# monkey0head/RePlay_cql

Measured on NVIDIA B200. Metric: CQL updates/sec (batch 1024), higher is better.
Workload: dtype f32 (f16x3: tensor-core fp16 hi/lo 3-term split with exact power-of-two row scales, fp32 accumulate, 1e-4 parity-gated)

## Files before the change

### replay_cql_b200/csrc/adam_pack.cuh

```cuda
#pragma once
#include "mlp_tc_h2.cuh"

namespace cql {
namespace tc {

struct AdamPackNet {
  float* p;
  float* m;
  float* v;
  const float* g;
  float* targ;
  uint8_t* fwd;
  uint8_t* fwd2;
  uint8_t* bwd;
  uint8_t* bwd2;
  uint8_t* tfwd;
  uint8_t* tfwd2;
  int* w2max;
};
struct AdamPackJobs {
  AdamPackNet n[CQL_MAX_CRITICS];
  int in_dim, out_dim;
  float lr, beta1, beta2, eps, tau;
  long long* step_inc;
  DpPeer dp;
  int dp_group;
  long long dp_off;
};

__device__ __forceinline__ float adam_one(float& p, float& m, float& v, float g, float step_size, float bc2s, float beta1,
                                          float beta2, float eps) {
  const float mi = m + (g - m) * (1.f - beta1);
  const float vi = v * beta2 + (1.f - beta2) * g * g;
  m = mi;
  v = vi;
  p = p - step_size * (mi / (sqrtf(vi) / bc2s + eps));
  return p;
}

__device__ __forceinline__ void store_chunk(const float (&x)[8], float s, uint8_t* one, uint8_t* pair, int n, int kc) {
  uint32_t hi[4], lo[4];
#pragma unroll
  for (int i = 0; i < 4; ++i) split_h2(x[2 * i] * s, x[2 * i + 1] * s, hi[i], lo[i]);
  const uint4 h4 = make_uint4(hi[0], hi[1], hi[2], hi[3]), l4 = make_uint4(lo[0], lo[1], lo[2], lo[3]);
  uint8_t* b = one + (size_t)(n / HCfg::NS) * HCfg::B_BYTES + chunk_off(HCfg::NS, n % HCfg::NS, kc);
  *reinterpret_cast<uint4*>(b) = h4;
  *reinterpret_cast<uint4*>(b + HCfg::B_TERM_BYTES) = l4;
  if (pair != nullptr) {
    *reinterpret_cast<uint4*>(pair + pair_chunk_off(n, kc, 0)) = h4;
    *reinterpret_cast<uint4*>(pair + pair_chunk_off(n, kc, 1)) = l4;
  }
}

constexpr int AP_ROWS = 8;
constexpr int AP_W2_BLOCKS = H / AP_ROWS;

__global__ void __launch_bounds__(1024, 1) k_adam_pack(const AdamPackJobs jobs, const StepInfo* __restrict__ si) {
  grid_dep_wait();
  __shared__ float tile[AP_ROWS][H + 4];
  __shared__ int wm[16];
  const AdamPackNet nt = jobs.n[blockIdx.y];
  const int in_dim = jobs.in_dim, out_dim = jobs.out_dim;
  const float step_size = (float)((double)jobs.lr / si->bc1), bc2s = (float)si->bc2_sqrt;
  const int slot_rd = (int)(si->step % 3), slot_acc = (int)((si->step + 1) % 3), slot_clr = (int)((si->step + 2) % 3);
  const int tid = threadIdx.x, lane = tid & 31;
  const bool dp = jobs.dp.world > 1;
  const long long dpb = jobs.dp_off + (long long)blockIdx.y * NET_STRIDE;
  DpSlices sl{};
  if (dp) {
    sl = dp_slices(jobs.dp, jobs.dp_off, (long long)gridDim.y * NET_STRIDE);
    dp_ll_owner_reduce(jobs.dp, jobs.dp_group, sl, jobs.n[0].g, ((long long)blockIdx.y * gridDim.x + blockIdx.x) * blockDim.x + tid,
                       (long long)gridDim.x * gridDim.y * blockDim.x);
  }
  if (blockIdx.x < AP_W2_BLOCKS) {
    __shared__ float gw2[AP_ROWS][H];
    __shared__ float rmax[AP_ROWS][4], rmaxt[AP_ROWS][4];
    const int r8 = tid >> 7, c2 = tid & 127;
    const int n = blockIdx.x * AP_ROWS + r8;
    const size_t off = (size_t)off_W2(in_dim) + (size_t)n * H + c2 * 2;
    const float w2max_prev = __int_as_float(nt.w2max[slot_rd]);
    float2 g = *reinterpret_cast<const float2*>(nt.g + off);
    float2 m = *reinterpret_cast<const float2*>(nt.m + off), v = *reinterpret_cast<const float2*>(nt.v + off);
    float2 p = *reinterpret_cast<const float2*>(nt.p + off), t = *reinterpret_cast<const float2*>(nt.targ + off);
    if (dp) {
      if ((c2 & 3) == 0) {
        float4 g0 = *reinterpret_cast<const float4*>(nt.g + off), g1 = *reinterpret_cast<const float4*>(nt.g + off + 4);
        dp_ll_mean8(jobs.dp, jobs.dp_group, sl, dpb + (long long)off, g0, g1);
        *reinterpret_cast<float4*>(&gw2[r8][c2 * 2]) = g0;
        *reinterpret_cast<float4*>(&gw2[r8][c2 * 2 + 4]) = g1;
      }
      __syncthreads();
      g = *reinterpret_cast<const float2*>(&gw2[r8][c2 * 2]);
    }
    adam_one(p.x, m.x, v.x, g.x, step_size, bc2s, jobs.beta1, jobs.beta2, jobs.eps);
    adam_one(p.y, m.y, v.y, g.y, step_size, bc2s, jobs.beta1, jobs.beta2, jobs.eps);
    t.x = t.x * (1.f - jobs.tau) + jobs.tau * p.x;
    t.y = t.y * (1.f - jobs.tau) + jobs.tau * p.y;
    *reinterpret_cast<float2*>(nt.m + off) = m;
    *reinterpret_cast<float2*>(nt.v + off) = v;
    *reinterpret_cast<float2*>(nt.p + off) = p;
    *reinterpret_cast<float2*>(nt.targ + off) = t;
    *reinterpret_cast<float2*>(&tile[r8][c2 * 2]) = p;
    float mx = fmaxf(fabsf(p.x), fabsf(p.y)), mt = fmaxf(fabsf(t.x), fabsf(t.y));
#pragma unroll
    for (int o = 16; o > 0; o >>= 1) {
      mx = fmaxf(mx, __shfl_xor_sync(0xffffffffu, mx, o));
      mt = fmaxf(mt, __shfl_xor_sync(0xffffffffu, mt, o));
    }
    if (lane == 0) { rmax[r8][(tid >> 5) & 3] = mx; rmaxt[r8][(tid >> 5) & 3] = mt; }
    __syncthreads();
    mx = fmaxf(fmaxf(rmax[r8][0], rmax[r8][1]), fmaxf(rmax[r8][2], rmax[r8][3]));
    mt = fmaxf(fmaxf(rmaxt[r8][0], rmaxt[r8][1]), fmaxf(rmaxt[r8][2], rmaxt[r8][3]));
    float s, inv_s, st, inv_st;
    pow2_scale(mx, s, inv_s);
    pow2_scale(mt, st, inv_st);
    {
// ... 9 lines not shown
      if (nt.fwd2 != nullptr) {
        *reinterpret_cast<uint32_t*>(nt.fwd2 + pair_chunk_off(n, kc, 0) + piece) = hi;
        *reinterpret_cast<uint32_t*>(nt.fwd2 + pair_chunk_off(n, kc, 1) + piece) = lo;
      }
      if (nt.tfwd2 != nullptr) {
        *reinterpret_cast<uint32_t*>(nt.tfwd2 + pair_chunk_off(n, kc, 0) + piece) = thi;
        *reinterpret_cast<uint32_t*>(nt.tfwd2 + pair_chunk_off(n, kc, 1) + piece) = tlo;
      }
    }
    if (c2 == 0) {
      reinterpret_cast<HMeta*>(nt.fwd + HCfg::META_OFF)->inv_s[n] = inv_s;
      reinterpret_cast<HMeta*>(nt.tfwd + HCfg::META_OFF)->inv_s[n] = inv_st;
      if (nt.fwd2) reinterpret_cast<HMeta*>(nt.fwd2 + H2Cfg::META_OFF)->inv_s[n] = inv_s;
      if (nt.tfwd2) reinterpret_cast<HMeta*>(nt.tfwd2 + H2Cfg::META_OFF)->inv_s[n] = inv_st;
      atomicMax(&nt.w2max[slot_acc], __float_as_int(mx));
    }
    if (tid < H) {
      const float bound = 2.f * (w2max_prev + 4.f * jobs.lr);
      float sT, inv_sT;
      pow2_scale(bound, sT, inv_sT);
      const int np = tid;
      float x[8];
#pragma unroll
      for (int i = 0; i < 8; ++i) x[i] = tile[i][np];
      store_chunk(x, sT, nt.bwd, nt.bwd2, np, (int)blockIdx.x);
      if (blockIdx.x == 0) {
        reinterpret_cast<HMeta*>(nt.bwd + HCfg::META_OFF)->inv_s[np] = inv_sT;
        if (nt.bwd2) reinterpret_cast<HMeta*>(nt.bwd2 + H2Cfg::META_OFF)->inv_s[np] = inv_sT;
      }
    }
    if (dp) dp_consume_done(jobs.dp, jobs.dp_group, gridDim.x * gridDim.y);
    return;
  }
  if (tid >= 256) return;
  if (tid < 16) wm[tid] = 0;
  if (tid == 0) nt.w2max[slot_clr] = 0;
  __syncthreads();
  __shared__ float gsm[2048];
  const int w2_lo = off_W2(in_dim), w2_hi = w2_lo + H * H;
  if (dp) {
    {
      const int c = tid * 8;
      const int idx = c < w2_lo ? c : c + H * H;
      if (idx + 7 < NET_STRIDE) {
        float4 a = *reinterpret_cast<const float4*>(nt.g + idx), b = *reinterpret_cast<const float4*>(nt.g + idx + 4);
        dp_ll_mean8(jobs.dp, jobs.dp_group, sl, dpb + idx, a, b);
        *reinterpret_cast<float4*>(gsm + c) = a;
        *reinterpret_cast<float4*>(gsm + c + 4) = b;
      }
    }
    __syncthreads();
  }
  auto grad_of = [&](int idx) { return dp ? gsm[idx < w2_lo ? idx : idx - H * H] : nt.g[idx]; };
  const int k = tid;
  int idxs[8];
  int n_idx = 0;
  for (int c = 0; c < in_dim; ++c) idxs[n_idx++] = off_W1(in_dim) + k * in_dim + c;
  idxs[n_idx++] = off_b1(in_dim) + k;
  idxs[n_idx++] = off_b2(in_dim) + k;
  for (int o = 0; o < out_dim; ++o) idxs[n_idx++] = off_W3(in_dim) + o * H + k;
  const bool has_b3 = tid < out_dim;
  const int ib3 = off_b3(in_dim, out_dim) + tid;
  float gv[9], pv[9], mv[9], vv[9], tv[9];
#pragma unroll
  for (int i = 0; i < 8; ++i)
    if (i < n_idx) { gv[i] = grad_of(idxs[i]); pv[i] = nt.p[idxs[i]]; mv[i] = nt.m[idxs[i]]; vv[i] = nt.v[idxs[i]]; tv[i] = nt.targ[idxs[i]]; }
  if (has_b3) { gv[8] = grad_of(ib3); pv[8] = nt.p[ib3]; mv[8] = nt.m[ib3]; vv[8] = nt.v[ib3]; tv[8] = nt.targ[ib3]; }
#pragma unroll
  for (int i = 0; i < 9; ++i)
    if (i < n_idx || (i == 8 && has_b3)) {
      adam_one(pv[i], mv[i], vv[i], gv[i], step_size, bc2s, jobs.beta1, jobs.beta2, jobs.eps);
// ... 52 lines not shown
```

### replay_cql_b200/csrc/capi.cu

```cuda
#include <cstring>
#include <cstdio>
#include <algorithm>
#include "engine.cuh"
#include "update.cuh"
#include "score.cuh"
#include "tc_selftest.cuh"
#include "score_tc.cuh"
#include "score_tc_h.cuh"
#include "topk_staged.cuh"
#include "metrics.cuh"
#include "dp_peer.cuh"
#include "mma_bench.cuh"

using namespace cql;

struct cql_handle {
  Handle h;
  cudaGraphExec_t graph_exec = nullptr;
  cudaStream_t graph_stream = nullptr;
  int64_t graph_launches = 0;
  cudaGraphExec_t batch_graph[2] = {nullptr, nullptr};
  cudaStream_t batch_graph_stream[2] = {nullptr, nullptr};
  int64_t batch_graph_launches[2] = {0, 0};
  void* sbuf[8] = {nullptr, nullptr, nullptr, nullptr, nullptr, nullptr, nullptr, nullptr};
// ... 155 lines not shown
  h.XT = h.dalloc<float4>(B);
  h.QT = h.dalloc<float>((size_t)C * B);
  h.XP = h.dalloc<float4>(B);
  h.QP = h.dalloc<float>((size_t)C * B);
  h.h2P = h.dalloc<float>((size_t)C * tB * H * BM);
  h.dQP = h.dalloc<float>((size_t)C * B);
  h.dXP = h.dalloc<float4>((size_t)C * B);
  h.dOutA = h.dalloc<float>(2 * (size_t)B);
  h.perb = h.dalloc<float>(4 * (size_t)B);
  h.pairv = h.dalloc<float>(4 * (size_t)C * B);
  h.loss_sums = h.dalloc<float>(16);
  h.actor_part = h.dalloc<float>((size_t)((B + 127) / 128) * 4 + 4);
  h.splitsC = std::max(1, std::min(tC, (2 * h.num_sms) / (4 * C)));
  h.splitsA = std::max(1, std::min(tB, (2 * h.num_sms) / 4));
  h.smallC = h.dalloc<float>((size_t)C * tC * SMALL_STRIDE);
  h.smallA = h.dalloc<float>((size_t)tB * SMALL_STRIDE);
  h.pw2C = h.dalloc<float>((size_t)C * h.splitsC * H * H);
  h.pw2A = h.dalloc<float>((size_t)h.splitsA * H * H);
  if (cfg->precision != CQL_PREC_FP32) {
    const bool bf = cfg->precision == CQL_PREC_BF16, f16 = cfg->precision == CQL_PREC_F16X3;
    h.packed_net_bytes = f16 ? tc::HCfg::PACKED_NET_BYTES : (bf ? tc::Cfg<false>::PACKED_NET_BYTES : tc::Cfg<true>::PACKED_NET_BYTES);
    h.packed_net_bytes_bwd = f16 ? tc::HCfg::PACKED_NET_BYTES : (bf ? tc::Cfg<false>::PACKED_NET_BYTES : tc::Cfg<true>::PACKED_NET_BYTES);
    h.packed_fwd = h.dalloc<uint8_t>((size_t)(2 + 2 * C) * h.packed_net_bytes);
    const int slices = f16 ? tc::HCfg::SLICES : (bf ? tc::Cfg<false>::SLICES : tc::Cfg<true>::SLICES);
    h.part_floats = (size_t)C * std::max(slices, (int)tc::H2Cfg::PARTS) * ((size_t)B * (2 * n3 + 2)) * 2 + 4096;
    h.part = h.dalloc<float>(h.part_floats);
    h.tc_slices = slices;
    h.packed_bwd = h.dalloc<uint8_t>((size_t)(1 + C) * h.packed_net_bytes_bwd);
    if (f16) {
      h.packed_net_bytes2 = tc::H2Cfg::PACKED_NET_BYTES;
      h.packed_fwd2 = h.dalloc<uint8_t>((size_t)(2 + 2 * C) * h.packed_net_bytes2);
      h.packed_bwd2 = h.dalloc<uint8_t>((size_t)(1 + C) * h.packed_net_bytes2);
      h.w2max = h.dalloc<int>((size_t)(2 + 2 * C) * 4);
      if (const char* sw = std::getenv("CQL_PAIR_SWAP")) h.pair_swap_b = std::atoi(sw);
    }
    h.slots1 = (f16 ? tc::HCfg::NEW : 4) * h.num_sms;
    h.splits_tc = h.num_sms;
    h.small1 = h.dalloc<float>((size_t)C * h.slots1 * SMALL_STRIDE);
    h.small2 = h.dalloc<float>((size_t)C * h.splits_tc * SMALL_STRIDE);
    h.pw2_tc = h.dalloc<float>((size_t)(h.num_sms + C) * H * H);
    h.dX_part = h.dalloc<float4>((size_t)C * std::max(slices, 8) * B);
    h.b2_tickets = h.dalloc<unsigned int>((size_t)CQL_MAX_CRITICS * 64 + 64);
  }
  float sc[SCALAR_SLOT] = {0};
  sc[0] = logf(cfg->initial_temperature);
  sc[1] = logf(cfg->initial_alpha);
  CQL_CUDA(cudaMemcpy(h.scalars(), sc, sizeof(sc), cudaMemcpyHostToDevice));
}

void destroy_graph(cql_handle* ch) {
  if (ch->graph_exec) { cudaGraphExecDestroy(ch->graph_exec); ch->graph_exec = nullptr; }
  for (auto& g : ch->batch_graph) if (g) { cudaGraphExecDestroy(g); g = nullptr; }
  if (ch->step_graph) { cudaGraphExecDestroy(ch->step_graph); ch->step_graph = nullptr; }
}

template <typename F>
int guarded(cql_handle* ch, F&& f) {
  if (!ch) { g_create_error = "NULL handle"; return 1; }
  struct DeviceScope {
    int prev = -1;
    ~DeviceScope() { if (prev >= 0) cudaSetDevice(prev); }
  } scope;
  try {
    int cur = -1;
    if (cudaGetDevice(&cur) == cudaSuccess && cur != ch->h.cfg.device) scope.prev = cur;
    CQL_CUDA(cudaSetDevice(ch->h.cfg.device));
// ... 856 lines not shown
```

### replay_cql_b200/csrc/engine.cuh

```cuda
#pragma once
#include <vector>
#include <string>
#include "common.cuh"
#include "mlp_simt.cuh"
#include "dp_peer.cuh"
#include <nvtx3/nvToolsExt.h>

namespace cql {

constexpr int N_NOISE_PARTS = 8;

struct StepInfo {
  double bc1, bc2_sqrt;
  long long step;
};

struct NvtxRange {
  explicit NvtxRange(const char* name) { nvtxRangePushA(name); }
  ~NvtxRange() { nvtxRangePop(); }
  NvtxRange(const NvtxRange&) = delete;
  NvtxRange& operator=(const NvtxRange&) = delete;
};

struct MdpSession;
// ... 45 lines not shown
  float* h2C = nullptr;
  float* dQ = nullptr;
  float4* XT = nullptr;
  float* QT = nullptr;
  float4* XP = nullptr;
  float* QP = nullptr;
  float* h2P = nullptr;
  float* dQP = nullptr;
  float4* dXP = nullptr;
  float* dOutA = nullptr;
  float* perb = nullptr;
  float* pairv = nullptr;
  float* loss_sums = nullptr;
  float* actor_part = nullptr;
  float* smallC = nullptr;
  float* smallA = nullptr;
  float* pw2C = nullptr;
  float* pw2A = nullptr;
  int splitsC = 1, splitsA = 1;

  uint8_t* packed_fwd = nullptr;
  size_t packed_net_bytes = 0;
  size_t packed_net_bytes_bwd = 0;
  float* part = nullptr;
  size_t part_floats = 0;
  uint8_t* packed_bwd = nullptr;
  float* small1 = nullptr;
  float* small2 = nullptr;
  float* pw2_tc = nullptr;
  float4* dX_part = nullptr;
  unsigned int* b2_tickets = nullptr;
  int slots1 = 0, splits_tc = 0, tc_slices = 1;
  int last_dx_parts = 0;
  uint8_t* packed_fwd2 = nullptr;
  uint8_t* packed_bwd2 = nullptr;
  size_t packed_net_bytes2 = 0;
  DpPeer dp;
  bool dp_fused = false;
  int* w2max = nullptr;
  int pair_swap_b = 0;

  bool timing = false;
  cudaEvent_t ev[16] = {};

  MdpSession* mdp = nullptr;
  uint8_t* mdp_ring = nullptr;
  std::vector<void*> allocs;

  template <typename T>
  T* dalloc(size_t count) {
    void* p = nullptr;
    CQL_CUDA(cudaMalloc(&p, count * sizeof(T)));
    CQL_CUDA(cudaMemset(p, 0, count * sizeof(T)));
    allocs.push_back(p);
    return reinterpret_cast<T*>(p);
  }
  void free_all() {
    for (void* p : allocs) cudaFree(p);
    allocs.clear();
    if (mdp) { mdp_session_free(mdp); mdp = nullptr; }
    if (mdp_ring) { cudaFreeHost(mdp_ring); mdp_ring = nullptr; }
    if (table) { cudaFree(table); table = nullptr; table_cap = 0; }
    if (metrics_host) { cudaFreeHost(metrics_host); metrics_host = nullptr; }
    if (batch_host) { cudaFreeHost(batch_host); batch_host = nullptr; }
    if (noise_host) { cudaFreeHost(noise_host); noise_host = nullptr; }
    if (own_stream) { cudaStreamDestroy(own_stream); own_stream = nullptr; }
    if (side_stream) { cudaStreamDestroy(side_stream); side_stream = nullptr; }
    if (ev_fork) { cudaEventDestroy(ev_fork); ev_fork = nullptr; }
    if (ev_join) { cudaEventDestroy(ev_join); ev_join = nullptr; }
    for (auto& e : ev) if (e) { cudaEventDestroy(e); e = nullptr; }
  }

// ... 36 lines not shown
```

### replay_cql_b200/csrc/mlp_tc_bwd1.cuh

```cuda
#pragma once
#include "mlp_tc.cuh"
#include "mlp_tc_ts.cuh"

namespace cql {
namespace tc {

struct Bwd1Job {
  const float4* X;
  const float* dOut;
  const float* h2;
  const float* params;
  const uint8_t* packedT;
  float* small1;
  float4* dX_part;
  int rows, n_nets, slots;
  const float* q_part = nullptr;
  int q_parts = 0;
  float dq_scale = 0.f;
};
template <int IN, int OUT>
__device__ __forceinline__ float actor_dq_of(const Bwd1Job& jb, int net_i, int r) {
  constexpr int MAXP = 8;
  int arg = 0;
  float qm = 0.f;
  for (int c = 0; c < jb.n_nets; ++c) {
    float part[MAXP];
#pragma unroll
    for (int p = 0; p < MAXP; ++p)
      if (p < jb.q_parts) part[p] = __ldg(jb.q_part + ((size_t)c * jb.q_parts + p) * jb.rows + r);
    const float bias = __ldg(jb.params + (size_t)c * NET_STRIDE + off_b3(IN, OUT));
    float v = 0.f;
#pragma unroll
    for (int p = 0; p < MAXP; ++p)
      if (p < jb.q_parts) v += part[p];
    const float q = v + bias;
    if (c == 0 || q < qm) { qm = q; arg = c; }
  }
  return net_i == arg ? jb.dq_scale : 0.f;
}

__device__ __forceinline__ float warp_reduce_scatter32(float (&v)[32]) {
  const int lane = threadIdx.x & 31;
#pragma unroll
  for (int off = 16; off >= 1; off >>= 1) {
    const bool upper = (lane & off) != 0;
#pragma unroll
    for (int i = 0; i < off; ++i) {
      const float send = upper ? v[i] : v[i + off];
      const float keep = upper ? v[i + off] : v[i];
      v[i] = keep + __shfl_xor_sync(0xffffffffu, send, off);
    }
  }
// ... 465 lines not shown
      tc_fence_before();
      __syncwarp();
      if (lane == 0) mbar_arrive(&tempty[acc]);
      if (DX && row < jb.rows)
        jb.dX_part[((size_t)net_i * C::SLICES + slice) * jb.rows + row] = make_float4(dx0, dx1, dx2, 0.f);
      ++tcount;
    }
    flush(cur_pair);
  }
  tc_fence_before();
  __syncthreads();
  if (warp == C::MMA_WARP) tmem_dealloc(tmem, C::TMEM_ALLOC);
}

__device__ __forceinline__ float4 sum_strided4(const float* __restrict__ p, int n, size_t stride) {
  float4 s0 = make_float4(0.f, 0.f, 0.f, 0.f), s1 = s0, s2 = s0, s3 = s0;
  int i = 0;
  for (; i + 4 <= n; i += 4) {
    const float4 a = __ldg(reinterpret_cast<const float4*>(p + (size_t)i * stride));
    const float4 b = __ldg(reinterpret_cast<const float4*>(p + (size_t)(i + 1) * stride));
    const float4 c = __ldg(reinterpret_cast<const float4*>(p + (size_t)(i + 2) * stride));
    const float4 d = __ldg(reinterpret_cast<const float4*>(p + (size_t)(i + 3) * stride));
    s0.x += a.x; s0.y += a.y; s0.z += a.z; s0.w += a.w;
    s1.x += b.x; s1.y += b.y; s1.z += b.z; s1.w += b.w;
    s2.x += c.x; s2.y += c.y; s2.z += c.z; s2.w += c.w;
    s3.x += d.x; s3.y += d.y; s3.z += d.z; s3.w += d.w;
  }
  for (; i < n; ++i) {
    const float4 a = __ldg(reinterpret_cast<const float4*>(p + (size_t)i * stride));
    s0.x += a.x; s0.y += a.y; s0.z += a.z; s0.w += a.w;
  }
  return make_float4((s0.x + s1.x) + (s2.x + s3.x), (s0.y + s1.y) + (s2.y + s3.y), (s0.z + s1.z) + (s2.z + s3.z),
                     (s0.w + s1.w) + (s2.w + s3.w));
}

__global__ void __launch_bounds__(256) k_reduce_grads_tc(const float* __restrict__ small1, int slots1,
                                                         const float* __restrict__ small2, const float* __restrict__ pw2,
                                                         int splits, int in_dim, int out_dim, float* __restrict__ grads,
                                                         int w2_group = 1, const DpPeer dp = DpPeer{}, int dp_group = 0,
                                                         long long dp_off = 0) {
  tc::grid_dep_wait();
 
  __shared__ float4 part[8][32];
  const int net = blockIdx.y;
  const int g = threadIdx.x & 31, chunk = threadIdx.x >> 5;
  const int idx = (blockIdx.x * 32 + g) * 4;
  const int w2_lo = off_W2(in_dim), w2_hi = w2_lo + H * H, total = net_floats(in_dim, out_dim);
  float4 s = make_float4(0.f, 0.f, 0.f, 0.f);
  if (idx < NET_STRIDE) {
    const float* base = nullptr;
    int n = 0;
    size_t stride = 0;
    if (idx >= w2_lo && idx < w2_hi) {
      base = pw2 + (size_t)net * splits * H * H + (idx - w2_lo); n = (splits + w2_group - 1) / w2_group; stride = (size_t)w2_group * H * H;
    } else if (idx < w2_lo) {
      base = small1 + (size_t)net * slots1 * SMALL_STRIDE + idx; n = slots1; stride = SMALL_STRIDE;
    } else if (idx < total) {
      base = small2 + (size_t)net * splits * SMALL_STRIDE + (idx - H * H); n = splits; stride = SMALL_STRIDE;
    }
    const int per = (n + 7) / 8, lo = chunk * per, hi = min(n, lo + per);
    if (base != nullptr && hi > lo) s = sum_strided4(base + (size_t)lo * stride, hi - lo, stride);
  }
  part[chunk][g] = s;
  __syncthreads();
  if (chunk == 0 && idx < NET_STRIDE) {
    float4 t = part[0][g];
// ... 11 lines not shown
```

### replay_cql_b200/csrc/mlp_tc_h.cuh

```cuda
#pragma once
#include <cuda_fp16.h>
#include "mlp_tc.cuh"
#include "mlp_tc_bwd1.cuh"
#include "mlp_tc_bwd2.cuh"

namespace cql {
namespace tc {

template <int NEW_, int NS_ = 128>
struct HCfgT {
  static constexpr int ES = 2, EPC = 8, UK = 16;
  static constexpr int NS = NS_;
  static constexpr int SLICES = H / NS;
  static constexpr int NPW = 16;
  static constexpr int KC = 64;
  static constexpr int STAGES = 4;
  static constexpr int NCHUNK = H / KC;
  static constexpr int KPW = KC / (NPW / 4);
  static constexpr int NEW = NEW_;
  static constexpr int MMA_WARP = NEW + NPW;
  static constexpr int THREADS = (NEW + 1 + NPW) * 32;
  static constexpr int PROD_THREADS = NPW * 32;
  static constexpr uint32_t B_TERM_BYTES = NS * H * ES;
  static constexpr uint32_t B_BYTES = 2 * B_TERM_BYTES;
// ... 401 lines not shown
  float4* ebs = reinterpret_cast<float4*>(sm + C::OFF_EB);
  float* invs = reinterpret_cast<float*>(sm + C::OFF_W1 + H * 8);
  uint64_t* bars = reinterpret_cast<uint64_t*>(sm + C::OFF_BAR);
  uint64_t* full = bars;
  uint64_t* empty = bars + C::STAGES;
  uint64_t* tfull = bars + 2 * C::STAGES;
  uint64_t* tempty = tfull + 2;
  uint64_t* bload = tempty + 2;
  uint64_t* drain = bload + 1;
  uint32_t* slot = reinterpret_cast<uint32_t*>(sm + C::OFF_SLOT);

  const int tid = threadIdx.x, warp = tid >> 5, lane = tid & 31;
  const int tiles = (jb.rows + TM - 1) / TM;
  const int tiles64 = (jb.rows + 63) / 64;
  const int total = jb.n_nets * C::SLICES * tiles;
  const int item_lo = (int)((long long)total * blockIdx.x / gridDim.x);
  const int item_hi = (int)((long long)total * (blockIdx.x + 1) / gridDim.x);

  if (warp == C::MMA_WARP) {
    tmem_alloc(slot, C::TMEM_ALLOC);
    if (lane == 0) {
      for (int s = 0; s < C::STAGES; ++s) { mbar_init(&full[s], C::NPW); mbar_init(&empty[s], 1); }
      for (int q = 0; q < 2; ++q) { mbar_init(&tfull[q], 1); mbar_init(&tempty[q], 4); }
      mbar_init(bload, 1);
      mbar_init(drain, 1);
      fence_mbar_init();
    }
  }
  tc_fence_before();
  __syncthreads();
  tc_fence_after();
  const uint32_t tmem = *slot;
  grid_dep_wait();

  if (warp == C::MMA_WARP) {
    const uint32_t idesc = instr_desc(FMT_F16, TM, C::NS);
    const uint32_t b_lbo = C::NS * 16;
    const uint32_t b_base = smem_u32(Bs);
    int cur_pair = -1;
    uint32_t it = 0, nb = 0, nd = 0, tcount = 0;
    for (int item = item_lo; item < item_hi; ++item) {
      const int pair = item / tiles;
      if (pair != cur_pair) {
        if (cur_pair >= 0) { if (elect_one()) umma_commit(drain); __syncwarp(); mbar_wait(drain, nd & 1); ++nd; }
        if (elect_one()) load_operand_slice<C>(Bs, jb.packedT + (size_t)(pair / C::SLICES) * HCfg::PACKED_NET_BYTES, pair % C::SLICES, bload);
        __syncwarp();
        mbar_wait(bload, nb & 1);
        ++nb;
        cur_pair = pair;
      }
      const uint32_t acc = tcount & 1;
      mbar_wait(&tempty[acc], ((tcount >> 1) & 1) ^ 1);
      tc_fence_after();
      const uint32_t d_tmem = tmem + acc * C::NS;
      for (int c = 0; c < C::NCHUNK; ++c, ++it) {
        const uint32_t s = it % C::STAGES;
        mbar_wait(&full[s], (it / C::STAGES) & 1);
        tc_fence_after();
        if (elect_one()) {
          const uint32_t a_stage = tmem + C::A_COL0 + s * C::A_STAGE_COLS;
#pragma unroll
          for (int j = 0; j < C::KC / C::UK; ++j) {
            const uint32_t g = c * (C::KC / C::UK) + j;
            const uint64_t b_hi = smem_desc(b_base + 2 * g * b_lbo, b_lbo, 128);
            const uint64_t b_lo = smem_desc(b_base + C::B_TERM_BYTES + 2 * g * b_lbo, b_lbo, 128);
            const uint32_t a_hi = a_stage + j * 8, a_lo = a_hi + C::A_LO_COLS;
// ... 494 lines not shown
```

### replay_cql_b200/csrc/mlp_tc_h2.cuh

```cuda
#pragma once
#include "mlp_tc_h.cuh"

namespace cql {
namespace tc {

__device__ __forceinline__ uint32_t cluster_ctarank() {
  uint32_t r;
  asm volatile("mov.u32 %0, %%cluster_ctarank;" : "=r"(r));
  return r;
}
__device__ __forceinline__ void cluster_sync_all() {
  asm volatile("barrier.cluster.arrive.release.aligned;" ::: "memory");
  asm volatile("barrier.cluster.wait.acquire.aligned;" ::: "memory");
}
__device__ __forceinline__ void mbar_arrive_cluster(uint64_t* bar, uint32_t cta) {
  asm volatile(
      "{\n\t.reg .b32 ra;\n\tmapa.shared::cluster.u32 ra, %0, %1;\n\t"
      "mbarrier.arrive.shared::cluster.b64 _, [ra];\n\t}" ::"r"(smem_u32(bar)),
      "r"(cta)
      : "memory");
}
__device__ __forceinline__ void mbar_wait_cluster(uint64_t* bar, uint32_t parity) { mbar_wait(bar, parity); }
__device__ __forceinline__ void tmem_alloc2(uint32_t* smem_slot, uint32_t ncols) {
  asm volatile("tcgen05.alloc.cta_group::2.sync.aligned.shared::cta.b32 [%0], %1;" ::"r"(smem_u32(smem_slot)), "r"(ncols)
// ... 443 lines not shown
  uint64_t* tempty = tfull + 2;
  uint64_t* bload = tempty + 2;
  uint64_t* bready = bload + 1;
  uint64_t* drain = bready + 1;
  uint32_t* slot = reinterpret_cast<uint32_t*>(sm + C::OFF_SLOT);

  const int tid = threadIdx.x, warp = tid >> 5, lane = tid & 31;
  const uint32_t rank = cluster_ctarank();
  const bool leader = rank == 0;
  const int cluster_id = blockIdx.x >> 1, n_clusters = gridDim.x >> 1;
  const int tiles = pair_tiles(jb.rows);
  const int tiles64 = (jb.rows + 63) / 64;
  const int total = jb.n_nets * tiles;
  const int item_lo = (int)((long long)total * cluster_id / n_clusters);
  const int item_hi = (int)((long long)total * (cluster_id + 1) / n_clusters);

  if (warp == C::MMA_WARP) {
    tmem_alloc2(slot, 512);
    if (lane == 0) {
      for (int s = 0; s < C::STAGES; ++s) { mbar_init(&full[s], 2 * C::NPW); mbar_init(&empty[s], 1); }
      for (int a = 0; a < 2; ++a) { mbar_init(&tfull[a], 1); mbar_init(&tempty[a], 2 * C::NEW); }
      mbar_init(bload, 1);
      mbar_init(bready, 2);
      mbar_init(drain, 1);
      fence_mbar_init();
    }
  }
  tc_fence_before();
  __syncthreads();
  cluster_sync_all();
  tc_fence_after();
  const uint32_t tmem = *slot;
  grid_dep_wait();

  if (warp == C::MMA_WARP) {
    const uint32_t idesc = instr_desc(FMT_F16, C::TMP, C::NP);
    const uint32_t b_lbo = C::NLOC * 16;
    const uint32_t b_base = smem_u32(Bs);
    int cur_net = -1;
    uint32_t nb = 0, nd = 0, tcount = 0;
    for (int item = item_lo; item < item_hi; ++item) {
      const int net_i = item / tiles;
      if (net_i != cur_net) {
        if (cur_net >= 0) {
          if (leader && elect_one()) umma_commit2(drain, 3);
          __syncwarp();
          mbar_wait_cluster(drain, nd & 1);
          ++nd;
        }
        const uint8_t* src = jb.packedT + (size_t)net_i * C::PACKED_NET_BYTES + (size_t)(rank ^ (uint32_t)swap_b) * C::B_BYTES;
        if (elect_one()) {
          mbar_arrive_expect_tx(bload, C::B_BYTES);
          for (uint32_t o = 0; o < C::B_BYTES; o += 32768) bulk_g2s(Bs + o, src + o, 32768, bload);
        }
        __syncwarp();
        mbar_wait(bload, nb & 1);
        if (elect_one()) mbar_arrive_cluster(bready, 0);
        __syncwarp();
        if (leader) mbar_wait_cluster(bready, nb & 1);
        ++nb;
        cur_net = net_i;
      }
      if (!leader) continue;
      for (int p = 0; p < C::PASSES; ++p) {
        mbar_wait_cluster(&tempty[p], (tcount & 1) ^ 1);
        tc_fence_after();
// ... 545 lines not shown
```

### replay_cql_b200/csrc/update.cuh

```cuda
#pragma once
#include <algorithm>
#include <utility>
#include <cstdlib>
#include "engine.cuh"
#include "mlp_tc.cuh"
#include "mlp_tc_ts.cuh"
#include <type_traits>
#include "mlp_tc_bwd1.cuh"
#include "mlp_tc_bwd2.cuh"
#include "mlp_tc_h.cuh"
#include "mlp_tc_h2.cuh"
#include "adam_pack.cuh"

namespace cql {

__host__ __device__ inline uint32_t mix32(uint32_t x) {
  x ^= x >> 16; x *= 0x7feb352du; x ^= x >> 15; x *= 0x846ca68bu; x ^= x >> 16;
  return x;
}
__host__ __device__ inline uint64_t feistel_perm(uint64_t x, uint64_t n, uint64_t key) {
  int bits = 2;
  while (bits < 62 && (1ull << bits) < n) bits += 2;
  const int hb = bits / 2;
  const uint64_t mask = (1ull << hb) - 1;
// ... 703 lines not shown
  }
  if (jobs_h.n) {
    launch_pdl(tc::k_pack_multi_h, dim3(dim3(H * 32 / 256, jobs_h.n)), dim3(256), 0, st, jobs_h, 2);
    CQL_LAUNCH_CHECK(h);
    tc::PackJobs jp{};
    for (int i = 0; i < n_slots; ++i) {
      const int slot = slots[i];
      const bool is_actor = slot == slot_actor() || slot == slot_targ_actor(h->C);
      if (is_actor) continue;
      jp.j[jp.n++] = {h->net_params(slot), h->packed_fwd2 + (size_t)slot * h->packed_net_bytes2, 3, 0};
      if (slot <= h->C) jp.j[jp.n++] = {h->net_params(slot), h->packed_bwd2 + (size_t)slot * h->packed_net_bytes2, 3, 1};
    }
    if (jp.n) {
      launch_pdl(tc::k_pack_pair_h, dim3(dim3(H * 32 / 256, jp.n)), dim3(256), 0, st, jp, 2);
      CQL_LAUNCH_CHECK(h);
    }
  }
  if (jobs.n == 0) return;
  if (h->cfg.precision != CQL_PREC_BF16) {
    const int chunks = H * (H / tc::Cfg<true>::EPC);
    tc::k_pack_multi<true><<<dim3((chunks + 255) / 256, jobs.n), 256, 0, st>>>(jobs);
  } else {
    const int chunks = H * (H / tc::Cfg<false>::EPC);
    tc::k_pack_multi<false><<<dim3((chunks + 255) / 256, jobs.n), 256, 0, st>>>(jobs);
  }
  CQL_LAUNCH_CHECK(h);
}
inline void pack_weights(Handle* h, int slot, int n_slots, int , cudaStream_t st) {
  int slots[8];
  for (int i = 0; i < n_slots; ++i) slots[i] = slot + i;
  pack_slots(h, slots, n_slots, st);
}

template <bool TF32, int IN, int OUT, bool WGRADS, bool DX, bool F16X3 = false>
inline void launch_bwd_tc(Handle* h, const BwdJob& jb, float* grads_out, cudaStream_t st, int mark_mid = -1, int mark_end = -1) {
  using C = std::conditional_t<F16X3, tc::HCfg, tc::Cfg<TF32>>;
  const int slot = (int)((jb.params - h->params) / NET_STRIDE);
  const int tiles = (jb.rows + tc::TM - 1) / tc::TM;
  const int items = jb.n_nets * C::SLICES * tiles;
  bool pair = false;
  if constexpr (F16X3) {
    static const bool no_pair = std::getenv("CQL_NO_PAIR") != nullptr || std::getenv("CQL_NO_PAIR_BWD1") != nullptr;
    pair = !no_pair && IN == 3 && jb.n_nets * ((jb.rows + 2 * tc::TM - 1) / (2 * tc::TM)) >= h->num_sms / 2;
  }
  bool small = false;
  if constexpr (F16X3) {
    static const bool no_small = std::getenv("CQL_NO_SMALL") != nullptr;
    small = !pair && !no_small && items * 2 <= h->num_sms;
  }
  const int n_slices = small ? tc::HCfgS::SLICES : C::SLICES;
  const int items_s = jb.n_nets * n_slices * tiles;
  static const bool no_fork = std::getenv("CQL_NO_FORK") != nullptr;
  static const int big_fork = std::getenv("CQL_BIG_FORK") ? std::atoi(std::getenv("CQL_BIG_FORK")) : -1;
  const int fork_pairs = big_fork >= 0 ? big_fork : (h->num_sms / 2) * 30 / 74;
  const int clusters1 = (pair && WGRADS && fork_pairs > 0 && fork_pairs < h->num_sms / 2 && !no_fork && !h->timing && h->side_stream != nullptr)
                            ? fork_pairs : h->num_sms / 2;
  const int grid1 = pair ? 2 * clusters1 : (items_s < h->num_sms ? items_s : h->num_sms);
  h->last_dx_parts = jb.n_nets * (pair ? (int)tc::H2Cfg::PARTS : n_slices);
  const int slots1 = (F16X3 ? 2 : 4) * grid1;
  if (WGRADS) CQL_CUDA(cudaMemsetAsync(h->small1, 0, (size_t)jb.n_nets * slots1 * SMALL_STRIDE * sizeof(float), st));
  tc::Bwd1Job j1{jb.X, jb.dOut, jb.h2, jb.params,
                 pair ? h->packed_bwd2 + (size_t)slot * h->packed_net_bytes2 : h->packed_bwd + (size_t)slot * h->packed_net_bytes_bwd,
                 h->small1, DX ? h->dX_part : nullptr, jb.rows, jb.n_nets, slots1};
  j1.q_part = jb.q_part; j1.q_parts = jb.q_parts; j1.dq_scale = jb.dq_scale;
  constexpr int RS2 = F16X3 ? tc::B2HCfg::RS : tc::B2Cfg<TF32>::RS;
  const int n_stage = (jb.rows + RS2 - 1) / RS2;
  int splits = h->num_sms / jb.n_nets;
  if (splits > n_stage) splits = n_stage;
  if (splits > h->splits_tc) splits = h->splits_tc;
  if (splits < 1) splits = 1;
  bool pair2 = false;
  if constexpr (F16X3) {
    static const bool no_pair2 = std::getenv("CQL_NO_PAIR") != nullptr || std::getenv("CQL_NO_PAIR_BWD2") != nullptr;
    static const bool no_pair2_small = std::getenv("CQL_NO_PAIR_BWD2_SMALL") != nullptr;
    pair2 = !no_pair2 && (pair || !no_pair2_small);
    if (pair2) splits = std::max(1, std::min(n_stage, (h->num_sms / 2) / jb.n_nets));
    if (pair2 && pair && clusters1 < h->num_sms / 2) splits = std::max(1, (h->num_sms / 2 - clusters1) / jb.n_nets);
  }
  const bool fork = WGRADS && !no_fork && !h->timing && h->side_stream != nullptr &&
                    grid1 + (pair2 ? 2 : 1) * splits * jb.n_nets <= h->num_sms;
  cudaStream_t st2 = st;
  if (fork) {
    CQL_CUDA(cudaEventRecord(h->ev_fork, st));
    CQL_CUDA(cudaStreamWaitEvent(h->side_stream, h->ev_fork, 0));
    st2 = h->side_stream;
  }
  if constexpr (F16X3) {
    if (pair) launch_pdl_pair(tc::tc_bwd1_h2_kernel<IN, OUT, WGRADS, DX>, clusters1, dim3(tc::H2Cfg::THREADS), tc::H2B1Cfg::SMEM_BYTES, st, j1, h->pair_swap_b);
    else if (small) launch_pdl(tc::tc_bwd1_h_kernel<IN, OUT, WGRADS, DX, tc::HCfgS>, dim3(grid1), dim3(tc::HCfgS::THREADS), tc::HCfgS::SMEM_BYTES, st, j1);
    else launch_pdl(tc::tc_bwd1_h_kernel<IN, OUT, WGRADS, DX>, dim3(grid1), dim3(tc::HCfg::THREADS), tc::HCfg::SMEM_BYTES, st, j1);
  } else if constexpr (TF32)
    tc::tc_bwd1_ts_kernel<IN, OUT, WGRADS, DX><<<grid1, tc::TsCfg::THREADS, tc::TsCfg::SMEM_BYTES, st>>>(j1);
  else
    tc::tc_bwd1_kernel<TF32, IN, OUT, WGRADS, DX><<<grid1, tc::Pipe<TF32, tc::BWD1_NPW>::THREADS, tc::FwdSmem<TF32, tc::BWD1_NPW>::BYTES, st>>>(j1);
  CQL_LAUNCH_CHECK(h);
  if (mark_mid >= 0) mark(h, st, mark_mid);
  if (!WGRADS) return;
  tc::Bwd2Job j2{jb.X, jb.dOut, jb.h2, jb.params, h->pw2_tc, h->small2, jb.rows, jb.n_nets, splits};
  constexpr bool GROUP_SUM = false;
  if (F16X3 && GROUP_SUM) j2.tickets = h->b2_tickets;
  if constexpr (F16X3) {
    if (pair2) {
      static const bool no_pdl_env = std::getenv("CQL_NO_PDL") != nullptr;
      cudaLaunchConfig_t cfg{};
      cfg.gridDim = dim3(2 * splits, jb.n_nets); cfg.blockDim = dim3(tc::B2PCfg::THREADS); cfg.dynamicSmemBytes = tc::B2PCfg::BYTES; cfg.stream = st2;
      cudaLaunchAttribute attr[1];
      attr[0].id = cudaLaunchAttributeProgrammaticStreamSerialization;
      attr[0].val.programmaticStreamSerializationAllowed = 1;
      cfg.attrs = attr;
      cfg.numAttrs = (no_pdl_env || g_timing_no_pdl) ? 0 : 1;
      CQL_CUDA(cudaLaunchKernelEx(&cfg, tc::tc_bwd2_h2_kernel<IN, OUT>, j2));
    } else {
      launch_pdl(tc::tc_bwd2_h_kernel<IN, OUT>, dim3(splits, jb.n_nets), dim3(tc::B2HCfg::THREADS), tc::B2HCfg::BYTES, st2, j2);
    }
  } else
    tc::tc_bwd2_kernel<TF32, IN, OUT><<<dim3(splits, jb.n_nets), tc::B2_THREADS, tc::B2Cfg<TF32>::BYTES, st2>>>(j2);
  CQL_LAUNCH_CHECK(h);
  if (fork) {
    CQL_CUDA(cudaEventRecord(h->ev_join, st2));
    CQL_CUDA(cudaStreamWaitEvent(st, h->ev_join, 0));
  }
  if (mark_end >= 0) mark(h, st, mark_end);
  if (!skip_launch(64))
    launch_pdl(tc::k_reduce_grads_tc, dim3(dim3((NET_STRIDE / 4 + 31) / 32, jb.n_nets)), dim3(256), 0, st, h->small1, slots1, h->small2, h->pw2_tc,
                                                                                  splits, IN, OUT, grads_out,
                                                                                  (F16X3 && GROUP_SUM) ? tc::B2H_GROUP : 1,
                                                                                  h->dp_fused ? h->dp : DpPeer{}, IN == 3 ? 1 : 2,
                                                                                  (long long)(IN == 3 ? NET_STRIDE : 0));
  CQL_LAUNCH_CHECK(h);
}

inline void adam_pack(Handle* h, int first_slot, int n_nets, int in_dim, int out_dim, float lr, cudaStream_t st, bool last = false) {
  const cql_config& c = h->cfg;
  tc::AdamPackJobs j{};
  j.in_dim = in_dim; j.out_dim = out_dim;
  j.lr = lr; j.beta1 = c.beta1; j.beta2 = c.beta2; j.eps = c.adam_eps; j.tau = c.tau;
  j.step_inc = last ? h->step_dev : nullptr;
  j.dp = h->dp_fused ? h->dp : DpPeer{};
  j.dp_group = in_dim == 3 ? 1 : 2;
  j.dp_off = (long long)first_slot * NET_STRIDE;
  for (int i = 0; i < n_nets; ++i) {
    const int slot = first_slot + i, tslot = slot + 1 + h->C;
    const bool critic = in_dim == 3;
    tc::AdamPackNet& n = j.n[i];
    n.p = h->net_params(slot);
    n.m = h->adam_m + (size_t)slot * NET_STRIDE;
    n.v = h->adam_v + (size_t)slot * NET_STRIDE;
    n.g = h->grads + (size_t)slot * NET_STRIDE;
    n.targ = h->net_params(tslot);
    n.fwd = h->packed_fwd + (size_t)slot * h->packed_net_bytes;
    n.bwd = h->packed_bwd + (size_t)slot * h->packed_net_bytes_bwd;
    n.tfwd = h->packed_fwd + (size_t)tslot * h->packed_net_bytes;
    n.fwd2 = critic ? h->packed_fwd2 + (size_t)slot * h->packed_net_bytes2 : nullptr;
    n.bwd2 = critic ? h->packed_bwd2 + (size_t)slot * h->packed_net_bytes2 : nullptr;
    n.tfwd2 = critic ? h->packed_fwd2 + (size_t)tslot * h->packed_net_bytes2 : nullptr;
    n.w2max = h->w2max + slot * 4;
  }
  if (!skip_launch(128))
    launch_pdl(tc::k_adam_pack, dim3(tc::AP_W2_BLOCKS + 1, n_nets), dim3(1024), 0, st, j, h->stepinfo);
  CQL_LAUNCH_CHECK(h);
}

inline void pack_all_weights(Handle* h, cudaStream_t st) {
  if (h->cfg.precision == CQL_PREC_F16X3) {
    tc::k_w2max_init<<<2 + 2 * h->C, 256, 0, st>>>(h->params, 2 + 2 * h->C, h->w2max);
    CQL_LAUNCH_CHECK(h);
  }
  pack_weights(h, slot_actor(), 1, 2, st);
  pack_weights(h, slot_critic(0), h->C, 3, st);
  pack_weights(h, slot_targ_actor(h->C), 1, 2, st);
  pack_weights(h, slot_targ_critic(h->C, 0), h->C, 3, st);
}

template <int IN, int OUT, bool WGRADS, bool DX>
inline void launch_bwd1(Handle* h, const BwdJob& jb, cudaStream_t st) {
  mlp_bwd1_kernel<IN, OUT, WGRADS, DX><<<tiles_of(jb.rows) * jb.n_nets, NT, BWD1_SMEM, st>>>(jb);
  CQL_LAUNCH_CHECK(h);
}

template <int IN, int OUT>
inline void launch_bwd2(Handle* h, const BwdJob& jb, cudaStream_t st) {
  mlp_bwd2_kernel<IN, OUT><<<dim3(4, jb.splits, jb.n_nets), NT, BWD2_SMEM, st>>>(jb);
  CQL_LAUNCH_CHECK(h);
}

inline LossConsts loss_consts(const Handle* h) {
  const cql_config& c = h->cfg;
  return LossConsts{h->B, h->n, h->C, c.gamma, c.conservative_weight, c.alpha_threshold,
                    c.temp_lr, c.alpha_lr, c.beta1, c.beta2, c.adam_eps};
}

constexpr int TIMED_FWD_REPS = 4;
// ... 195 lines not shown
```

Baseline: 4600.

## Fold gradient partial reduction into Adam-pack kernel and zero slots in bwd1

The separate k_reduce_grads_tc launch is dropped in the f16x3 single-device path. The Adam-pack kernel now sums the per-split W2 partials and the small-parameter slot partials itself, writes the gradient, and applies Adam. Small parameters are spread over many blocks, with a ticket-based last-block reduction for the weight maxima that go into the packed metadata. The cudaMemset of the small1 slots is replaced by zeroing inside the bwd1 kernel. This saves a kernel launch, a memset and a round trip of the gradients through global memory, at the cost of extra cross-block atomics and more work inside the Adam kernel.

```diff
diff --git a/replay_cql_b200/csrc/adam_pack.cuh b/replay_cql_b200/csrc/adam_pack.cuh
--- a/replay_cql_b200/csrc/adam_pack.cuh
+++ b/replay_cql_b200/csrc/adam_pack.cuh
@@ -8,7 +8,7 @@
   float* p;
   float* m;
   float* v;
-  const float* g;
+  float* g;
   float* targ;
   uint8_t* fwd;
   uint8_t* fwd2;
@@ -26,6 +26,11 @@
   DpPeer dp;
   int dp_group;
   long long dp_off;
+  const float* small1;
+  const float* small2;
+  const float* pw2;
+  int slots1, splits;
+  int* wmax_acc;
 };
 
 __device__ __forceinline__ float adam_one(float& p, float& m, float& v, float g, float step_size, float bc2s, float beta1,
@@ -54,10 +59,81 @@
 
 constexpr int AP_ROWS = 8;
 constexpr int AP_W2_BLOCKS = H / AP_ROWS;
+constexpr int AP_SMALL_E = 128;
+constexpr int ap_small_blocks(int in_dim, int out_dim) { return (net_floats(in_dim, out_dim) - H * H + AP_SMALL_E - 1) / AP_SMALL_E; }
+
+__device__ __forceinline__ void adam_small_fold(const AdamPackJobs& jobs, const AdamPackNet& nt, float step_size, float bc2s,
+                                             int slot_clr, int* wm) {
+  __shared__ float part[8][AP_SMALL_E];
+  __shared__ int last;
+  const int tid = threadIdx.x, in_dim = jobs.in_dim, out_dim = jobs.out_dim;
+  const int w2_lo = off_W2(in_dim), n_e = net_floats(in_dim, out_dim) - H * H;
+  const int s_blk = blockIdx.x - AP_W2_BLOCKS, n_blk = gridDim.x - AP_W2_BLOCKS;
+  const int el = tid % AP_SMALL_E, chunk = tid / AP_SMALL_E;
+  const int e = s_blk * AP_SMALL_E + el;
+  const int idx = e < w2_lo ? e : e + H * H;
+  const bool own = tid < AP_SMALL_E && e < n_e;
+  float p = 0.f, m = 0.f, v = 0.f, t = 0.f;
+  if (own) { p = nt.p[idx]; m = nt.m[idx]; v = nt.v[idx]; t = nt.targ[idx]; }
+  float s = 0.f;
+  if (e < n_e) {
+    if (e < w2_lo) s = chunk_sum8<float, 16>(jobs.small1 + (size_t)blockIdx.y * jobs.slots1 * SMALL_STRIDE + e, jobs.slots1, SMALL_STRIDE, chunk);
+    else s = chunk_sum8<float, 16>(jobs.small2 + (size_t)blockIdx.y * jobs.splits * SMALL_STRIDE + e, jobs.splits, SMALL_STRIDE, chunk);
+  }
+  part[chunk][el] = s;
+  if (tid < 16) wm[tid] = 0;
+  if (s_blk == 0 && tid == 0) {
+    nt.w2max[slot_clr] = 0;
+    if (jobs.step_inc != nullptr && blockIdx.y == 0) *jobs.step_inc += 1;
+  }
+  __syncthreads();
+  if (own) {
+    float g = part[0][el];
+#pragma unroll
+    for (int c = 1; c < 8; ++c) g += part[c][el];
+    nt.g[idx] = g;
+    m = __fmaf_rn(__fsub_rn(g, m), __fsub_rn(1.f, jobs.beta1), m);
+    v = __fmaf_rn(g, __fmul_rn(g, __fsub_rn(1.f, jobs.beta2)), __fmul_rn(jobs.beta2, v));
+    p = __fmaf_rn(-__fdiv_rn(m, __fadd_rn(__fdiv_rn(__fsqrt_rn(v), bc2s), jobs.eps)), step_size, p);
+    t = __fmaf_rn(t, __fsub_rn(1.f, jobs.tau), __fmul_rn(jobs.tau, p));
+    nt.p[idx] = p; nt.m[idx] = m; nt.v[idx] = v; nt.targ[idx] = t;
+    int slot = -1;
+    if (idx < off_b1(in_dim)) slot = idx % in_dim;
+    else if (idx < w2_lo) slot = 3;
+    else if (idx >= off_W3(in_dim) && idx < off_b3(in_dim, out_dim)) slot = 4 + (idx - off_W3(in_dim)) / H;
+    if (slot >= 0) {
+      atomicMax(&wm[slot], __float_as_int(fabsf(p)));
+      atomicMax(&wm[8 + slot], __float_as_int(fabsf(t)));
+    }
+  }
+  __syncthreads();
+  int* acc = jobs.wmax_acc + blockIdx.y * 16;
+  unsigned int* ticket = reinterpret_cast<unsigned int*>(jobs.wmax_acc + CQL_MAX_CRITICS * 16) + blockIdx.y;
+  if (tid < 16 && wm[tid] != 0) atomicMax(&acc[tid], wm[tid]);
+  __threadfence();
+  __syncthreads();
+  if (tid == 0) {
+    const unsigned int k = atomicAdd(ticket, 1u);
+    last = k == (unsigned int)n_blk - 1;
+    if (last) *ticket = 0;
+  }
+  __syncthreads();
+  if (!last) return;
+  __threadfence();
+  if (tid < 8) {
+    const float w = __int_as_float(atomicExch(&acc[tid], 0)), wt = __int_as_float(atomicExch(&acc[8 + tid], 0));
+    reinterpret_cast<HMeta*>(nt.fwd + HCfg::META_OFF)->wmax[tid] = w;
+    reinterpret_cast<HMeta*>(nt.bwd + HCfg::META_OFF)->wmax[tid] = w;
+    reinterpret_cast<HMeta*>(nt.tfwd + HCfg::META_OFF)->wmax[tid] = wt;
+    if (nt.fwd2) reinterpret_cast<HMeta*>(nt.fwd2 + H2Cfg::META_OFF)->wmax[tid] = w;
+    if (nt.bwd2) reinterpret_cast<HMeta*>(nt.bwd2 + H2Cfg::META_OFF)->wmax[tid] = w;
+    if (nt.tfwd2) reinterpret_cast<HMeta*>(nt.tfwd2 + H2Cfg::META_OFF)->wmax[tid] = wt;
+  }
+}
 
 __global__ void __launch_bounds__(1024, 1) k_adam_pack(const AdamPackJobs jobs, const StepInfo* __restrict__ si) {
   grid_dep_wait();
-  __shared__ float tile[AP_ROWS][H + 4];
+  __shared__ __align__(16) float tile[AP_ROWS][H + 4];
   __shared__ int wm[16];
   const AdamPackNet nt = jobs.n[blockIdx.y];
   const int in_dim = jobs.in_dim, out_dim = jobs.out_dim;
@@ -73,15 +149,21 @@
                        (long long)gridDim.x * gridDim.y * blockDim.x);
   }
   if (blockIdx.x < AP_W2_BLOCKS) {
-    __shared__ float gw2[AP_ROWS][H];
+    __shared__ __align__(16) float gw2[AP_ROWS][H];
     __shared__ float rmax[AP_ROWS][4], rmaxt[AP_ROWS][4];
     const int r8 = tid >> 7, c2 = tid & 127;
     const int n = blockIdx.x * AP_ROWS + r8;
     const size_t off = (size_t)off_W2(in_dim) + (size_t)n * H + c2 * 2;
     const float w2max_prev = __int_as_float(nt.w2max[slot_rd]);
-    float2 g = *reinterpret_cast<const float2*>(nt.g + off);
+    float2 g;
+    if (jobs.small1 == nullptr) g = *reinterpret_cast<const float2*>(nt.g + off);
     float2 m = *reinterpret_cast<const float2*>(nt.m + off), v = *reinterpret_cast<const float2*>(nt.v + off);
     float2 p = *reinterpret_cast<const float2*>(nt.p + off), t = *reinterpret_cast<const float2*>(nt.targ + off);
+    if (jobs.small1 != nullptr) {
+      g = reduce8<float2, 4>(jobs.pw2 + (size_t)blockIdx.y * jobs.splits * H * H + (off - off_W2(in_dim)), jobs.splits,
+                             (size_t)H * H);
+      *reinterpret_cast<float2*>(nt.g + off) = g;
+    }
     if (dp) {
       if ((c2 & 3) == 0) {
         float4 g0 = *reinterpret_cast<const float4*>(nt.g + off), g1 = *reinterpret_cast<const float4*>(nt.g + off + 4);
@@ -157,11 +239,15 @@
     if (dp) dp_consume_done(jobs.dp, jobs.dp_group, gridDim.x * gridDim.y);
     return;
   }
+  if (jobs.small1 != nullptr) {
+    adam_small_fold(jobs, nt, step_size, bc2s, slot_clr, wm);
+    return;
+  }
   if (tid >= 256) return;
   if (tid < 16) wm[tid] = 0;
   if (tid == 0) nt.w2max[slot_clr] = 0;
   __syncthreads();
-  __shared__ float gsm[2048];
+  __shared__ __align__(16) float gsm[2048];
   const int w2_lo = off_W2(in_dim), w2_hi = w2_lo + H * H;
   if (dp) {
     {
diff --git a/replay_cql_b200/csrc/capi.cu b/replay_cql_b200/csrc/capi.cu
--- a/replay_cql_b200/csrc/capi.cu
+++ b/replay_cql_b200/csrc/capi.cu
@@ -211,6 +211,7 @@
       h.packed_fwd2 = h.dalloc<uint8_t>((size_t)(2 + 2 * C) * h.packed_net_bytes2);
       h.packed_bwd2 = h.dalloc<uint8_t>((size_t)(1 + C) * h.packed_net_bytes2);
       h.w2max = h.dalloc<int>((size_t)(2 + 2 * C) * 4);
+      h.ap_wmax = h.dalloc<int>((size_t)CQL_MAX_CRITICS * 17);
       if (const char* sw = std::getenv("CQL_PAIR_SWAP")) h.pair_swap_b = std::atoi(sw);
     }
     h.slots1 = (f16 ? tc::HCfg::NEW : 4) * h.num_sms;
diff --git a/replay_cql_b200/csrc/engine.cuh b/replay_cql_b200/csrc/engine.cuh
--- a/replay_cql_b200/csrc/engine.cuh
+++ b/replay_cql_b200/csrc/engine.cuh
@@ -101,12 +101,14 @@
   unsigned int* b2_tickets = nullptr;
   int slots1 = 0, splits_tc = 0, tc_slices = 1;
   int last_dx_parts = 0;
+  int last_slots1 = 0, last_splits = 0;
   uint8_t* packed_fwd2 = nullptr;
   uint8_t* packed_bwd2 = nullptr;
   size_t packed_net_bytes2 = 0;
   DpPeer dp;
   bool dp_fused = false;
   int* w2max = nullptr;
+  int* ap_wmax = nullptr;
   int pair_swap_b = 0;
 
   bool timing = false;
diff --git a/replay_cql_b200/csrc/mlp_tc_bwd1.cuh b/replay_cql_b200/csrc/mlp_tc_bwd1.cuh
--- a/replay_cql_b200/csrc/mlp_tc_bwd1.cuh
+++ b/replay_cql_b200/csrc/mlp_tc_bwd1.cuh
@@ -17,7 +17,19 @@
   const float* q_part = nullptr;
   int q_parts = 0;
   float dq_scale = 0.f;
+  int zero_small1 = 0;
 };
+template <int IN>
+__device__ __forceinline__ void zero_small1_slots(const Bwd1Job& jb, int per_cta) {
+  if (!jb.zero_small1) return;
+  constexpr int NF4 = off_W2(IN) / 4;
+  for (int net = 0; net < jb.n_nets; ++net)
+    for (int s = 0; s < per_cta; ++s) {
+      float4* o = reinterpret_cast<float4*>(jb.small1 + ((size_t)net * jb.slots + (size_t)blockIdx.x * per_cta + s) * SMALL_STRIDE);
+      for (int f = threadIdx.x; f < NF4; f += blockDim.x) o[f] = make_float4(0.f, 0.f, 0.f, 0.f);
+    }
+  __syncthreads();
+}
 template <int IN, int OUT>
 __device__ __forceinline__ float actor_dq_of(const Bwd1Job& jb, int net_i, int r) {
   constexpr int MAXP = 8;
@@ -549,6 +561,54 @@
   }
   return make_float4((s0.x + s1.x) + (s2.x + s3.x), (s0.y + s1.y) + (s2.y + s3.y), (s0.z + s1.z) + (s2.z + s3.z),
                      (s0.w + s1.w) + (s2.w + s3.w));
+}
+
+__device__ __forceinline__ void vacc(float& s, float a) { s += a; }
+__device__ __forceinline__ void vacc(float2& s, float2 a) { s.x += a.x; s.y += a.y; }
+__device__ __forceinline__ float vfold(float a, float b, float c, float d) { return (a + b) + (c + d); }
+__device__ __forceinline__ float2 vfold(float2 a, float2 b, float2 c, float2 d) {
+  return make_float2((a.x + b.x) + (c.x + d.x), (a.y + b.y) + (c.y + d.y));
+}
+template <typename V> __device__ __forceinline__ V vld(const float* p);
+template <> __device__ __forceinline__ float vld<float>(const float* p) { return __ldg(p); }
+template <> __device__ __forceinline__ float2 vld<float2>(const float* p) { return __ldg(reinterpret_cast<const float2*>(p)); }
+template <typename V, int NPRE>
+__device__ __forceinline__ V sum_strided_pre(const float* __restrict__ p, int n, size_t stride) {
+  static_assert(NPRE % 4 == 0, "groups of four");
+  V s0{}, s1{}, s2{}, s3{};
+  if (n <= NPRE) {
+    V a[NPRE];
+#pragma unroll
+    for (int i = 0; i < NPRE; ++i)
+      if (i < n) a[i] = vld<V>(p + (size_t)i * stride);
+#pragma unroll
+    for (int i = 0; i < NPRE; i += 4)
+      if (i + 4 <= n) { vacc(s0, a[i]); vacc(s1, a[i + 1]); vacc(s2, a[i + 2]); vacc(s3, a[i + 3]); }
+#pragma unroll
+    for (int i = 0; i < NPRE; ++i)
+      if (i >= (n & ~3) && i < n) vacc(s0, a[i]);
+  } else {
+    int i = 0;
+    for (; i + 4 <= n; i += 4) {
+      const V a = vld<V>(p + (size_t)i * stride), b = vld<V>(p + (size_t)(i + 1) * stride);
+      const V c = vld<V>(p + (size_t)(i + 2) * stride), d = vld<V>(p + (size_t)(i + 3) * stride);
+      vacc(s0, a); vacc(s1, b); vacc(s2, c); vacc(s3, d);
+    }
+    for (; i < n; ++i) vacc(s0, vld<V>(p + (size_t)i * stride));
+  }
+  return vfold(s0, s1, s2, s3);
+}
+template <typename V, int NPRE>
+__device__ __forceinline__ V chunk_sum8(const float* __restrict__ p, int n, size_t stride, int chunk) {
+  const int per = (n + 7) / 8, lo = chunk * per, hi = min(n, lo + per);
+  return hi > lo ? sum_strided_pre<V, NPRE>(p + (size_t)lo * stride, hi - lo, stride) : V{};
+}
+template <typename V, int NPRE>
+__device__ __forceinline__ V reduce8(const float* __restrict__ p, int n, size_t stride) {
+  V t = chunk_sum8<V, NPRE>(p, n, stride, 0);
+#pragma unroll
+  for (int c = 1; c < 8; ++c) vacc(t, chunk_sum8<V, NPRE>(p, n, stride, c));
+  return t;
 }
 
 __global__ void __launch_bounds__(256) k_reduce_grads_tc(const float* __restrict__ small1, int slots1,
diff --git a/replay_cql_b200/csrc/mlp_tc_h.cuh b/replay_cql_b200/csrc/mlp_tc_h.cuh
--- a/replay_cql_b200/csrc/mlp_tc_h.cuh
+++ b/replay_cql_b200/csrc/mlp_tc_h.cuh
@@ -457,6 +457,7 @@
   tc_fence_after();
   const uint32_t tmem = *slot;
   grid_dep_wait();
+  if (WGRADS) zero_small1_slots<IN>(jb, 2);
 
   if (warp == C::MMA_WARP) {
     const uint32_t idesc = instr_desc(FMT_F16, TM, C::NS);
diff --git a/replay_cql_b200/csrc/mlp_tc_h2.cuh b/replay_cql_b200/csrc/mlp_tc_h2.cuh
--- a/replay_cql_b200/csrc/mlp_tc_h2.cuh
+++ b/replay_cql_b200/csrc/mlp_tc_h2.cuh
@@ -499,6 +499,7 @@
   tc_fence_after();
   const uint32_t tmem = *slot;
   grid_dep_wait();
+  if (WGRADS) zero_small1_slots<IN>(jb, 2);
 
   if (warp == C::MMA_WARP) {
     const uint32_t idesc = instr_desc(FMT_F16, C::TMP, C::NP);
diff --git a/replay_cql_b200/csrc/update.cuh b/replay_cql_b200/csrc/update.cuh
--- a/replay_cql_b200/csrc/update.cuh
+++ b/replay_cql_b200/csrc/update.cuh
@@ -759,6 +759,11 @@
   pack_slots(h, slots, n_slots, st);
 }
 
+inline bool fold_grads(const Handle* h) {
+  static const bool no_fold = std::getenv("CQL_NO_FOLD") != nullptr || std::getenv("CQL_NO_FUSED_ADAM") != nullptr;
+  return !no_fold && h->cfg.precision == CQL_PREC_F16X3 && h->cfg.world_size <= 1 && h->dp.world <= 1;
+}
+
 template <bool TF32, int IN, int OUT, bool WGRADS, bool DX, bool F16X3 = false>
 inline void launch_bwd_tc(Handle* h, const BwdJob& jb, float* grads_out, cudaStream_t st, int mark_mid = -1, int mark_end = -1) {
   using C = std::conditional_t<F16X3, tc::HCfg, tc::Cfg<TF32>>;
@@ -785,11 +790,13 @@
   const int grid1 = pair ? 2 * clusters1 : (items_s < h->num_sms ? items_s : h->num_sms);
   h->last_dx_parts = jb.n_nets * (pair ? (int)tc::H2Cfg::PARTS : n_slices);
   const int slots1 = (F16X3 ? 2 : 4) * grid1;
-  if (WGRADS) CQL_CUDA(cudaMemsetAsync(h->small1, 0, (size_t)jb.n_nets * slots1 * SMALL_STRIDE * sizeof(float), st));
+  const bool fold = F16X3 && WGRADS && fold_grads(h);
+  if (WGRADS && !fold) CQL_CUDA(cudaMemsetAsync(h->small1, 0, (size_t)jb.n_nets * slots1 * SMALL_STRIDE * sizeof(float), st));
   tc::Bwd1Job j1{jb.X, jb.dOut, jb.h2, jb.params,
                  pair ? h->packed_bwd2 + (size_t)slot * h->packed_net_bytes2 : h->packed_bwd + (size_t)slot * h->packed_net_bytes_bwd,
                  h->small1, DX ? h->dX_part : nullptr, jb.rows, jb.n_nets, slots1};
   j1.q_part = jb.q_part; j1.q_parts = jb.q_parts; j1.dq_scale = jb.dq_scale;
+  j1.zero_small1 = fold ? 1 : 0;
   constexpr int RS2 = F16X3 ? tc::B2HCfg::RS : tc::B2Cfg<TF32>::RS;
   const int n_stage = (jb.rows + RS2 - 1) / RS2;
   int splits = h->num_sms / jb.n_nets;
@@ -848,6 +855,11 @@
     CQL_CUDA(cudaStreamWaitEvent(st, h->ev_join, 0));
   }
   if (mark_end >= 0) mark(h, st, mark_end);
+  if (fold) {
+    h->last_slots1 = slots1;
+    h->last_splits = splits;
+    return;
+  }
   if (!skip_launch(64))
     launch_pdl(tc::k_reduce_grads_tc, dim3(dim3((NET_STRIDE / 4 + 31) / 32, jb.n_nets)), dim3(256), 0, st, h->small1, slots1, h->small2, h->pw2_tc,
                                                                                   splits, IN, OUT, grads_out,
@@ -883,8 +895,15 @@
     n.tfwd2 = critic ? h->packed_fwd2 + (size_t)tslot * h->packed_net_bytes2 : nullptr;
     n.w2max = h->w2max + slot * 4;
   }
+  const bool fold = fold_grads(h);
+  if (fold) {
+    j.small1 = h->small1; j.small2 = h->small2; j.pw2 = h->pw2_tc;
+    j.slots1 = h->last_slots1; j.splits = h->last_splits;
+    j.wmax_acc = h->ap_wmax;
+  }
+  const int blocks = tc::AP_W2_BLOCKS + (fold ? tc::ap_small_blocks(in_dim, out_dim) : 1);
   if (!skip_launch(128))
-    launch_pdl(tc::k_adam_pack, dim3(tc::AP_W2_BLOCKS + 1, n_nets), dim3(1024), 0, st, j, h->stepinfo);
+    launch_pdl(tc::k_adam_pack, dim3(blocks, n_nets), dim3(1024), 0, st, j, h->stepinfo);
   CQL_LAUNCH_CHECK(h);
 }
 
```

After: 4978 (median of 6 runs). +8.2%, better.
